# AnyLoc/Revisit-Anything

Hardware: AMD Instinct MI355X
Metric: query_images_per_sec (higher is better)
Workload: dtype f32

## Files before the change

### revisit-anything_amd/csrc/api.hip

```cpp
#include <stdarg.h>
#include <stdlib.h>
#include <string.h>

#include <cmath>
#include <mutex>
#include <utility>

#include <initializer_list>

#include "ctx.h"

int segvlad_ctx::fail(int code, const char* fmt, ...) {
  va_list ap;
  va_start(ap, fmt);
  vsnprintf(err, sizeof(err), fmt, ap);
  va_end(ap);
  return code;
}

bool sv_is_device_ptr(const void* p) {
  hipPointerAttribute_t a;
  memset(&a, 0, sizeof(a));
  hipError_t e = hipPointerGetAttributes(&a, p);
  if (e != hipSuccess) {
// ... 271 lines not shown
  if (!strcmp(key, "f16_gm")) return as_int(&o.f16_gm);
  if (!strcmp(key, "f16_walk")) return as_int(&o.f16_walk);
  if (!strcmp(key, "f16_deep_cfg")) return as_dev(&o.f16_deep_cfg, {-1, 4, 5});
  if (!strcmp(key, "f16_buf")) return as_dev(&o.f16_buf, {-1, 0});
  if (!strcmp(key, "tnk_gram")) return as_int(&o.tnk_gram);
  if (!strcmp(key, "tnk_fork")) return as_int(&o.tnk_fork);
  if (!strcmp(key, "x3_tile")) return as_int(&o.x3_tile);
  if (!strcmp(key, "x3_gm")) return as_int(&o.x3_gm);
  if (!strcmp(key, "search_stats")) return as_int(&o.search_stats);
  if (!strcmp(key, "knn_heuristic")) return as_int(&o.knn_heuristic);
  if (!strcmp(key, "assign_narrow")) return as_int(&o.assign_narrow);
  if (!strcmp(key, "agg_kpb")) return as_int(&o.agg_kpb);
  if (!strcmp(key, "pj_nw")) return as_int(&o.pj_nw);
  if (!strcmp(key, "pj_f16")) return as_int(&o.pj_f16);
  if (!strcmp(key, "cover_rows")) return as_int(&o.cover_rows);
  if (!strcmp(key, "small_plan")) return as_int(&o.small_plan);
  if (!strcmp(key, "small_tail")) return as_int(&o.small_tail);
  if (!strcmp(key, "small_head")) return as_int(&o.small_head);
  if (!strcmp(key, "batch_l0_f16")) return as_int(&o.batch_l0_f16);
  if (!strcmp(key, "level_carry")) return as_int(&o.level_carry);
  if (!strcmp(key, "f16_persist_wgs")) return as_int(&o.f16_persist_wgs);
  if (!strcmp(key, "debug_small_tail")) return as_int(&o.debug_small_tail);
  if (!strcmp(key, "refine_group")) return as_int(&o.refine_group);
  if (!strcmp(key, "query_group")) return as_int(&o.query_group);
  if (!strcmp(key, "group_fetch")) return as_int(&o.group_fetch);
  if (!strcmp(key, "debug_search")) return as_int(&o.debug_search);
  if (!strcmp(key, "debug_fail_search")) return as_int(&o.debug_fail_search);
  if (!strcmp(key, "guard_undersize")) {
    if (!ctx->guard) return ctx->fail(SEGVLAD_ERR_STATE, "set_option(guard_undersize): the context was not created under SEGVLAD_GUARD=1");
    const char* colon = strchr(value, ':');
// ... 353 lines not shown
```

### revisit-anything_amd/csrc/ctx.h

```cpp
#pragma once
#include <hip/hip_runtime.h>
#include <math.h>
#include <stdint.h>
#include <stdio.h>
#include <string.h>

#include <map>
#include <string>
#include <vector>

#include "../../include/segvlad.h"

#define SV_HIP(expr)                                                                              \
  do {                                                                                            \
    hipError_t _e = (expr);                                                                       \
    if (_e != hipSuccess) {                                                                       \
      return ctx->fail(SEGVLAD_ERR_HIP, "%s failed: %s (%s:%d)", #expr, hipGetErrorString(_e),    \
                       __FILE__, __LINE__);                                                       \
    }                                                                                             \
  } while (0)

#define SV_TRY(expr)          \
  do {                        \
    int _r = (expr);          \
// ... 94 lines not shown
  int agg_kpb = 4;
  int debug_fail_search = 0;
  int debug_search = 0;
  int debug_small_tail = 0;
  int batch_l0_f16 = 1;
  int level_carry = 1;
  int small_head = 1;
  int small_tail = 1;
  int small_plan = 1;
  int pj_f16 = 1;
  int pj_nw = 8;
  int refine_group = 1;
  int query_group = 0;
  int pca_path = 0;
  int cover_rows = 1;
  float vlad_soft_temp = 0.f;
  int vlad_soft_pooled = 0;
  int group_fetch = 0;
};

constexpr int SV_F16_KBLOCK = 1024;
inline int sv_f16_kblock(const SvOptions& o, int d) {
  if (o.f16_cfg == 300) return SV_F16_KBLOCK;
  return (o.f16_cfg < 0 && d >= 4096) ? SV_F16_KBLOCK : 0;
}
constexpr int SV_F16_KFLUSH = 64;
int sv_f16_eps_kblock(const SvOptions& o, int d);
inline bool sv_f16_bias_possible(const SvOptions& o, int64_t nq) { return nq > 128 && (o.f16_cfg < 0 || o.f16_cfg == 250 || o.f16_cfg == 300); }
enum class F16Kernel {
  None, BatchDefault, BatchComplement, BatchSmall, BatchUnbiased, BatchUnbiasedSmall, DeepFlush, DeepFlushComplement, DeepBlockedBuf, DeepBlocked,
// ... 269 lines not shown
int sv_launch_refine_grouped(segvlad_ctx* ctx, const float* Q, const float* R, int nq, int d, const float* qn, const float* rn,
                             const uint32_t* ref_cnt, const uint32_t* ref_id, int rcap, int k, float* d2_out, int64_t* idx_out,
                             int* launches, const uint32_t* only_rows = nullptr, int live_groups_hint = 0);
int sv_refine_group_stats(segvlad_ctx* ctx, int nq, int64_t* groups, int64_t* grouped, int64_t* union_sum);
int sv_row_norm_max(segvlad_ctx* ctx, const float* norms, int64_t n, float* out_host, bool finite_only = false);
int sv_row_norm_min(segvlad_ctx* ctx, const float* norms, int64_t n, float* out_host);
int sv_maxabs(segvlad_ctx* ctx, const float* x, int64_t n, float* out_host, bool finite_only = false, bool* nonfinite_host = nullptr);
int sv_maxabs_and_norm_min_begin(segvlad_ctx* ctx, const float* x, int64_t n, const float* norms, int64_t n_norms);
int sv_maxabs_and_norm_min_end(segvlad_ctx* ctx, int64_t n, int64_t n_norms, float* maxabs_host, float* norm_min_host, bool* nonfinite_host,
                               float* norm_max_host);
int sv_launch_split_f16x2(segvlad_ctx* ctx, const float* X, int64_t n_rows, int d, const float* sub, float scale, uint16_t* h1,
                          uint16_t* h2);
int sv_launch_gemm_f16x3(segvlad_ctx* ctx, const uint16_t* A1, const uint16_t* A2, const uint16_t* B1, const uint16_t* B2, int M,
                         int N, int Kd, float out_scale, const float* col_scale, float* C);
int sv_launch_gemm_f16x3_grouped(segvlad_ctx* ctx, const uint16_t* A1, const uint16_t* A2, const uint16_t* B1, const uint16_t* B2,
                                 int M_pad, int N, int Kd, int n_groups, const int32_t* tile_group, float out_scale, float* C);
int sv_launch_group_plan(segvlad_ctx* ctx, const int32_t* cov_cnt, int B, int K, int32_t* rowbase, int32_t* tile_group, int max_tiles);
int sv_launch_project_consts(segvlad_ctx* ctx, const float* comps, const float* mean, int P, int64_t KD, float* wmu );
int sv_launch_project_aggregate(segvlad_ctx* ctx, const float* Z, const float* wmu, const float* block_norms, const float* gscale,
                                const uint64_t* colmask, const int32_t* lab_off, const int32_t* rowbase, const int32_t* phys,
                                const int32_t* seg_off_dev, int B, int N, int K, int P, int SC, int S_max, const float* col_scale,
                                float* Y, float zscale);
int sv_launch_to_f16(segvlad_ctx* ctx, const float* X, int64_t n_elems, float scale, uint16_t* out);
int sv_launch_query_f16_small(segvlad_ctx* ctx, const float* X, int64_t n_elems, float db_scale, uint16_t* out, float* scales_dev,
                              float* qn_out, int nq, int d, uint32_t* zero, int zero_words);
int sv_launch_to_f16_devscale(segvlad_ctx* ctx, const float* X, int64_t n_elems, const float* scales_dev, uint16_t* out);
int sv_launch_f16_filter(segvlad_ctx* ctx, const uint16_t* Qh, const uint16_t* Rh, int M, int n_sample, int d, int b_stride,
                         float inv_scale, const float* qn, const float* rn, const float* thr, int64_t thr_ld, float eps_mult,
                         float c_eps, float rn_max, uint32_t* cand_cnt, float* cand_d2, uint32_t* cand_id, int cap, int skip = 0);
bool sv_f16_filter_skip_ok(const segvlad_ctx* ctx, int M, int64_t n_rows, int d);

int sv_launch_select_cand(segvlad_ctx* ctx, const uint32_t* cand_cnt, const float* cand_d2, const uint32_t* cand_id,
                          int nq, int cap, int k, float* d2_out, int64_t* idx_out, uint32_t* ovf_rows, uint32_t* ovf_count);
int sv_launch_select_topk(segvlad_ctx* ctx, const float* dist, int64_t ld, int nq, int64_t n, int k, float* d2_out,
                          int64_t* idx_out, int64_t out_ld, int64_t id_base);
int sv_launch_merge_topk(segvlad_ctx* ctx, const float* d2_parts, const int64_t* idx_parts, int nq, int cand, int k,
                         float* d2_out, int64_t* idx_out);
// ... 62 lines not shown
```

### revisit-anything_amd/csrc/describe.hip

```cpp
#include <cmath>
#include "ctx.h"


struct SegWalk { int S_max = 0; bool monotone = true; std::vector<int64_t> adj_off; };
static SegWalk walk_seg_offsets(const int32_t* seg_offsets, int B) {
  SegWalk w;
  w.adj_off.assign((size_t)B + 1, 0);
  for (int b = 0; b < B && w.monotone; ++b) {
    const int s = seg_offsets[b + 1] - seg_offsets[b];
    w.monotone = s >= 0;
    if (s > w.S_max) w.S_max = s;
    w.adj_off[b + 1] = w.adj_off[b] + (int64_t)s * s;
  }
  return w;
}

static int incidence_run(segvlad_ctx* ctx, const uint8_t* masks, int S, int Hm, int Wm, int H, int W, int patch, uint64_t* inc_bits,
                         double* centroids, bool want_centroids) {
  if (S < 0 || Hm <= 0 || Wm <= 0 || H <= 0 || W <= 0 || patch <= 0 || H / patch <= 0 || W / patch <= 0)
    return ctx->fail(SEGVLAD_ERR_ARG, "incidence: bad geometry S=%d masks %dx%d image %dx%d patch %d", S, Hm, Wm, H, W, patch);
  if (S == 0) return SEGVLAD_OK;
  if (!masks || !inc_bits || (want_centroids && !centroids)) return ctx->fail(SEGVLAD_ERR_ARG, "incidence: null pointer");
  const int N = (H / patch) * (W / patch), nw = (N + 63) / 64;
  const void* dm;
// ... 121 lines not shown
  p.xscale = sv_fp16_scale(bound);
  p.rows_pad = (((int64_t)B * N + 255) & ~255ll) + 256ll * K;
  if (ctx->pca_w_scale > 0.f) {
    const float zb = std::sqrt((float)D) * (16384.f / ctx->pca_w_scale) * (1.f + ctx->vocab_norm_max);
    if (std::isfinite(zb) && zb > 0.f) p.zscale = sv_fp16_scale(zb);
  }
  return p;
#undef PLAN_REFUSE
}

static int reserve_scratch(segvlad_ctx* ctx, const DescribePlan& p, DescribeIO& io) {
  const size_t B = p.B, N = p.N, D = p.D, K = p.K, P = p.P, S = p.S_tot;
  if (p.form == DescribeForm::Project) {
    SV_HIP(ctx->s_xh1.reserve((size_t)(p.rows_pad + 256) * D * 2));
    SV_HIP(ctx->s_xh2.reserve((size_t)(p.rows_pad + 256) * D * 2));
    SV_HIP(ctx->s_pz.reserve((size_t)p.rows_pad * P * sizeof(float)));
    SV_HIP(ctx->s_rowbase.reserve(B * K * sizeof(int32_t)));
    SV_HIP(ctx->s_tilegrp.reserve((size_t)(p.rows_pad >> 8) * sizeof(int32_t)));
    SV_HIP(ctx->s_phys.reserve(B * N * sizeof(int32_t)));
    SV_HIP(ctx->s_covcnt.reserve(B * K * sizeof(int32_t)));
    SV_HIP(ctx->s_bn.reserve(S * K * sizeof(float)));
  } else if (p.form == DescribeForm::Planes) {
    SV_HIP(ctx->s_xh1.reserve((size_t)sv_x3_rows(p.S_tot) * ctx->KD * 2));
    SV_HIP(ctx->s_xh2.reserve((size_t)sv_x3_rows(p.S_tot) * ctx->KD * 2));
  } else if (p.form == DescribeForm::PlainProjection && !io.out && S > 0) {
    SV_HIP(ctx->s_desc.reserve(S * ctx->KD * sizeof(float)));
    io.out = ctx->s_desc.as<float>();
  }
  SV_HIP(ctx->s_xt.reserve(B * N * D * sizeof(float)));
  SV_HIP(ctx->s_rnorm.reserve(B * N * sizeof(float)));
  if (!p.want_labels) SV_HIP(ctx->s_labels.reserve(B * N));
// ... 100 lines not shown
}

static int pass_project(segvlad_ctx* ctx, const DescribePlan& p, const DescribeIO& io) {
  float* bn = io.d_bn ? (float*)io.d_bn : ctx->s_bn.as<float>();
  uint16_t *h1 = ctx->s_xh1.as<uint16_t>(), *h2 = ctx->s_xh2.as<uint16_t>();
  {
    StageScope sc(ctx, "aggregate");
    SV_TRY(sv_launch_group_plan(ctx, ctx->s_covcnt.as<int32_t>(), p.B, p.K, ctx->s_rowbase.as<int32_t>(), ctx->s_tilegrp.as<int32_t>(),
                                (int)(p.rows_pad >> 8)));
    SV_TRY(sv_launch_token_norms(ctx, ctx->s_xt.as<float>(), ctx->s_colmask.as<uint64_t>(), ctx->vocab.as<float>(), p.K, p.D,
                                 ctx->s_segoff.as<int32_t>(), p.B, p.N, p.SC, bn, p.xscale, h1, h2, ctx->s_rowbase.as<int32_t>(),
                                 ctx->opt.debug_search == 7 ? -p.rows_pad : p.rows_pad, ctx->s_phys.as<int32_t>()));
    sc.count(2);
  }
  StageScope sc(ctx, "pca");
  SV_TRY(sv_launch_gemm_f16x3_grouped(ctx, h1, h2, ctx->pca_w1.as<uint16_t>(), ctx->pca_w2.as<uint16_t>(), (int)p.rows_pad, p.P, p.D, p.K,
                                      ctx->s_tilegrp.as<int32_t>(), 1.f / (p.xscale * ctx->pca_w_scale), ctx->s_pz.as<float>()));
  SV_TRY(sv_launch_project_aggregate(ctx, ctx->s_pz.as<float>(), ctx->pca_cproj.as<float>(), bn, ctx->s_gscale.as<float>(),
                                     ctx->s_colmask.as<uint64_t>(), ctx->s_laboff.as<int32_t>(), ctx->s_rowbase.as<int32_t>(),
                                     ctx->s_phys.as<int32_t>(), ctx->s_segoff.as<int32_t>(), p.B, p.N, p.K, p.P, p.SC, p.S_max,
                                     ctx->pca_scale.as<float>(), (float*)io.d_y, p.zscale));
  sc.count(2);
  return pass_normalize(ctx, p, io, sc);
}

static int join_mask_branch(segvlad_ctx* ctx) {
  if (!ctx->desc.side_pending) return SEGVLAD_OK;
  ctx->desc.side_pending = false;
  return sv_join_side(ctx);
}
static int run_describe(segvlad_ctx* ctx, const DescribePlan& p, DescribeIO& io) {
  SV_TRY(reserve_scratch(ctx, p, io));
  if (p.form == DescribeForm::Project && !ctx->pca_cproj_valid) {
    SV_HIP(ctx->pca_cproj.reserve((size_t)ctx->P * sizeof(float)));
    SV_TRY(sv_launch_project_consts(ctx, ctx->pca_comps.as<float>(), ctx->pca_mean.as<float>(), ctx->P, ctx->KD, ctx->pca_cproj.as<float>()));
    ctx->pca_cproj_valid = true;
// ... 284 lines not shown
```

### revisit-anything_amd/csrc/gemm_f16x3_kernels.hip

```cpp
#include <stdlib.h>

#include "ctx.h"

typedef float f32x4 __attribute__((ext_vector_type(4)));
typedef _Float16 f16x8 __attribute__((ext_vector_type(8)));
typedef const __attribute__((address_space(1))) void* gptr_t;
typedef __attribute__((address_space(3))) void* lptr_t;
#define MFMA_F16(a, b, c) __builtin_amdgcn_mfma_f32_16x16x32_f16((a), (b), (c), 0, 0, 0)

__global__ __launch_bounds__(256) void split_f16x2_kernel(const float* __restrict__ X, int64_t n_rows, int d,
                                                          const float* __restrict__ sub, float scale,
                                                          _Float16* __restrict__ h1, _Float16* __restrict__ h2) {
  typedef _Float16 h4 __attribute__((ext_vector_type(4)));
  const int64_t n4 = n_rows * (int64_t)(d >> 2);
  const int d4 = d >> 2;
  for (int64_t j = (int64_t)blockIdx.x * 256 + threadIdx.x; j < n4; j += (int64_t)gridDim.x * 256) {
    float4 v = reinterpret_cast<const float4*>(X)[j];
    if (sub) {
      const float4 s = reinterpret_cast<const float4*>(sub)[j % d4];
      v.x -= s.x;
      v.y -= s.y;
      v.z -= s.z;
      v.w -= s.w;
    }
// ... 25 lines not shown
__device__ __forceinline__ void wait_vm_lgkm0_() {
  if (N_ == 0) asm volatile("s_waitcnt vmcnt(0) lgkmcnt(0)" ::: "memory");
  else if (N_ == 2) asm volatile("s_waitcnt vmcnt(2) lgkmcnt(0)" ::: "memory");
  else if (N_ == 4) asm volatile("s_waitcnt vmcnt(4) lgkmcnt(0)" ::: "memory");
  else asm volatile("s_waitcnt vmcnt(8) lgkmcnt(0)" ::: "memory");
}

template <int BM, int BN, int WM, int WN>
__global__ __launch_bounds__(64 * WM * WN) void gemm_f16x3_kernel(const uint16_t* __restrict__ A1,
                                                                  const uint16_t* __restrict__ A2,
                                                                  const uint16_t* __restrict__ B1,
                                                                  const uint16_t* __restrict__ B2, int M, int N, int Kd,
                                                                  int tiles_m, int gm, int n_splits, int k_per_split, float out_scale,
                                                                  const float* __restrict__ col_scale,
                                                                  float* __restrict__ C, int64_t ldc,
                                                                  const int32_t* __restrict__ tile_group, int nkb_b) {
  constexpr int NW = WM * WN;
  constexpr int TM = BM / (16 * WM), TN = BN / (16 * WN);
  static_assert(TM == 4 && (TN == 8 || TN == 4), "wave tiles of 64 rows, 128 or 64 columns");
  constexpr int HBK = 32, RB = 64, RP = 16;
  constexpr int PA = BM * RB, PB = BN * RB;
  constexpr int JA = BM / RP / NW, JB = BN / RP / NW;
  static_assert(JA * RP * NW == BM && JB * RP * NW == BN, "tile/wave geometry");
  extern __shared__ __attribute__((aligned(16))) unsigned char lds[];
  int tm, tn, split;
  if (gm > 0) {
    const int b = blockIdx.x, xcd = b & 7, s = b >> 3, within = s & 31, u = (s >> 5) * 8 + xcd;
    const int gn = 32 / gm, sm_cnt = (tiles_m + gm - 1) / gm, tiles_n = (N + BN - 1) / BN;
    split = u % n_splits;
    const int r = u / n_splits;
    tm = (r % sm_cnt) * gm + within % gm;
// ... 102 lines not shown
#pragma unroll
        for (int nt = 0; nt < 4; ++nt) acc[mt][4 * h + nt] = MFMA_F16(a1[mt], b1[nt], acc[mt][4 * h + nt]);
    }
    wait_vm_lgkm0_<0>();
    __builtin_amdgcn_s_barrier();
    cur ^= 1;
  }

  if (n_splits > 1) C += (int64_t)split * M * ldc;
#pragma unroll
  for (int nt = 0; nt < TN; ++nt) {
    const int64_t col = n0 + wn * (16 * TN) + nt * 16 + i;
    if (col >= N) continue;
    const float cs = (n_splits > 1) ? 1.f : out_scale * (col_scale ? col_scale[col] : 1.f);
#pragma unroll
    for (int mt = 0; mt < TM; ++mt)
#pragma unroll
      for (int r = 0; r < 4; ++r) {
        const int64_t row = m0 + wm * (16 * TM) + mt * 16 + 4 * kq + r;
        if (row < M) C[row * ldc + col] = acc[mt][nt][r] * cs;
      }
  }
}

__global__ __launch_bounds__(256) void splitk_reduce_scale_kernel(const float* __restrict__ part, int splits, int64_t mn,
                                                                  int N, float out_scale,
                                                                  const float* __restrict__ col_scale,
                                                                  float* __restrict__ out) {
  const int64_t j = (int64_t)blockIdx.x * 256 + threadIdx.x;
  if (j >= mn) return;
  float s = part[j];
  for (int t = 1; t < splits; ++t) s += part[(int64_t)t * mn + j];
  const int col = (int)(j % N);
  out[j] = s * out_scale * (col_scale ? col_scale[col] : 1.f);
}

// ... 25 lines not shown
  const size_t lds = 2 * (size_t)(2 * BM * 64 + 2 * BN * 64);
  auto kern = gemm_f16x3_kernel<BM, BN, WM, WN>;
  if (lds > 64 * 1024)
    SV_HIP(sv_max_dyn_lds(reinterpret_cast<const void*>(kern), (size_t)lds));
  int gm = ctx->opt.x3_gm > 0 ? ctx->opt.x3_gm : 0;
  dim3 grid((unsigned)tiles, (unsigned)splits);
  if (gm > 0) {
    gm = gm >= 32 ? 32 : gm >= 16 ? 16 : gm >= 8 ? 8 : gm >= 4 ? 4 : gm >= 2 ? 2 : 1;
    while (gm < 32 && 32 / gm > tiles_n) gm <<= 1;
    while (gm > 1 && gm / 2 >= tiles_m) gm >>= 1;
    const int gn = 32 / gm;
    const int64_t units = (int64_t)((tiles_m + gm - 1) / gm) * ((tiles_n + gn - 1) / gn) * splits;
    grid = dim3((unsigned)((units + 7) / 8 * 8 * 32), 1);
  }
  hipLaunchKernelGGL(kern, grid, dim3(64 * WM * WN), lds, ctx->stream, A1, A2, B1, B2, M, N, Kd, tiles_m, gm, splits, k_per_split,
                     out_scale, col_scale, dst, (int64_t)N, (const int32_t*)nullptr, 0);
  SV_HIP(hipGetLastError());
  if (splits > 1) {
    const int64_t mn = (int64_t)M * N;
    hipLaunchKernelGGL(splitk_reduce_scale_kernel, dim3((unsigned)((mn + 255) / 256)), dim3(256), 0, ctx->stream, dst, splits, mn,
                       N, out_scale, col_scale, C);
    SV_HIP(hipGetLastError());
  }
  return SEGVLAD_OK;
}

int sv_launch_gemm_f16x3(segvlad_ctx* ctx, const uint16_t* A1, const uint16_t* A2, const uint16_t* B1, const uint16_t* B2, int M,
                         int N, int Kd, float out_scale, const float* col_scale, float* C) {
  if (M <= 0 || N <= 0) return SEGVLAD_OK;
  const bool big = ctx->opt.x3_tile ? (ctx->opt.x3_tile == 256) : (M >= 1024);
  if (big) return launch_x3<256, 256, 4, 2>(ctx, A1, A2, B1, B2, M, N, Kd, out_scale, col_scale, C);
  return launch_x3<128, 128, 2, 2>(ctx, A1, A2, B1, B2, M, N, Kd, out_scale, col_scale, C);
}

int sv_launch_gemm_f16x3_grouped(segvlad_ctx* ctx, const uint16_t* A1, const uint16_t* A2, const uint16_t* B1, const uint16_t* B2,
                                 int M_pad, int N, int Kd, int n_groups, const int32_t* tile_group, float out_scale, float* C) {
  if (M_pad <= 0 || N <= 0) return SEGVLAD_OK;
  constexpr int BM = 256, BN = 256;
  const int tiles_m = M_pad / BM, tiles_n = (N + BN - 1) / BN;
  const size_t lds = 2 * (size_t)(2 * BM * 64 + 2 * BN * 64);
  auto kern = gemm_f16x3_kernel<BM, BN, 4, 2>;
  SV_HIP(sv_max_dyn_lds(reinterpret_cast<const void*>(kern), (size_t)lds));
  const int rows_per_chunk = 32 / tiles_n > 0 ? 32 / tiles_n : 1;
  const int chunks = (tiles_m + rows_per_chunk - 1) / rows_per_chunk;
  const int64_t grid = (int64_t)((chunks + 7) / 8) * 8 * rows_per_chunk * tiles_n;
  hipLaunchKernelGGL(kern, dim3((unsigned)grid, 1), dim3(512), lds, ctx->stream, A1, A2, B1, B2, M_pad, N, Kd, tiles_m, 0,
                     1, Kd, out_scale, (const float*)nullptr, C, (int64_t)N, tile_group, n_groups * (Kd >> 5));
  SV_HIP(hipGetLastError());
  return SEGVLAD_OK;
}
```

### revisit-anything_amd/csrc/project_kernels.hip

```cpp
#include "ctx.h"
#include "group_tile_dev.h"

#define MFMA32(a, b, c) __builtin_amdgcn_mfma_f32_32x32x2f32((a), (b), (c), 0, 0, 0)

__global__ __launch_bounds__(1024) void group_plan_kernel(const int32_t* __restrict__ cov_cnt, int B, int K,
                                                          int32_t* __restrict__ rowbase, int32_t* __restrict__ tile_group,
                                                          int max_tiles) {
  __shared__ int32_t part[1024], base[257];
  const int nsl = 1024 / K;
  const int k = threadIdx.x % K, c = threadIdx.x / K;
  const int per = (B + nsl - 1) / nsl, b0 = c * per, b1 = min(B, b0 + per);
  const bool act = c < nsl;
  for (int t = threadIdx.x; t < max_tiles; t += blockDim.x) tile_group[t] = -1;
  int sum = 0;
  if (act)
    for (int b = b0; b < b1; ++b) sum += cov_cnt[(size_t)b * K + k];
  part[threadIdx.x] = act ? sum : 0;
  __syncthreads();
  if ((int)threadIdx.x < K) {
    int run = 0;
    for (int q = 0; q < nsl; ++q) {
      const int v = part[q * K + threadIdx.x];
      part[q * K + threadIdx.x] = run;
      run += v;
// ... 38 lines not shown
  for (int o = 128; o > 0; o >>= 1) {
    if ((int)threadIdx.x < o) red[threadIdx.x] += red[threadIdx.x + o];
    __syncthreads();
  }
  if (threadIdx.x == 0) wmu[p] = (float)red[0];
}

int sv_launch_project_consts(segvlad_ctx* ctx, const float* comps, const float* mean, int P, int64_t KD, float* wmu) {
  hipLaunchKernelGGL(project_consts_kernel, dim3(P), dim3(256), 0, ctx->stream, comps, mean, P, KD, wmu);
  SV_HIP(hipGetLastError());
  return SEGVLAD_OK;
}

constexpr int PJ_T = 32;

template <int NW, bool F16 = false>
__global__ __launch_bounds__(64 * NW) void project_aggregate_kernel(const float* __restrict__ Z, const float* __restrict__ wmu,
                                                                const float* __restrict__ bn, const float* __restrict__ gscale,
                                                                const uint64_t* __restrict__ colmask,
                                                                const int32_t* __restrict__ lab_off,
                                                                const int32_t* __restrict__ rowbase,
                                                                const int32_t* __restrict__ phys,
                                                                const int32_t* __restrict__ seg_off, int N, int K, int P, int SC,
                                                                int maxt, const float* __restrict__ col_scale,
                                                                float* __restrict__ Y, float zscale) {
  extern __shared__ __attribute__((aligned(16))) unsigned char smem[];
  typedef _Float16 f16x8 __attribute__((ext_vector_type(8)));
  static_assert(!F16 || NW == 8, "16-bit tile sums: the 8-wave workgroup");
  const int KS = K + 1 + (K & 1);
  float* ag = reinterpret_cast<float*>(smem);
  constexpr int NC = 32 * NW, NT_ = 64 * NW, C4W = NC / 4;
  float* zt = ag + 64 * KS;
  uint64_t* mk = reinterpret_cast<uint64_t*>(zt + 2 * PJ_T * NC);
  int32_t* tl_k = reinterpret_cast<int32_t*>(mk + 2 * PJ_T);
  int32_t* tl_j = tl_k + maxt;
  int32_t* tl_z = tl_j + maxt;
  int32_t* tl_n = tl_z + maxt;
  int32_t* phl = tl_n + maxt + K + 1;
  uint4* af = reinterpret_cast<uint4*>((reinterpret_cast<uintptr_t>(phl + N) + 15) & ~(uintptr_t)15);
  __shared__ int s_tiles;
  const int b = blockIdx.y, p0 = blockIdx.x * NC;
  const int tid = threadIdx.x, w = tid >> 6, l = tid & 63, i = l & 31, kk = l >> 5;
  const int s0 = seg_off[b], S = seg_off[b + 1] - s0;
  const int SCb = (S + 63) >> 6;
  const int32_t* lo = lab_off + (size_t)b * (K + 1);
  const int pcol = p0 + 32 * w + i;
  int32_t* tl_pre = tl_n + maxt;
  int my_o0 = 0, my_n = 0, my_g0 = 0;
  if (tid < K) {
    my_o0 = lo[tid];
    my_n = lo[tid + 1] - my_o0;
    my_g0 = rowbase[(size_t)b * K + tid];
    tl_pre[tid + 1] = (my_n + PJ_T - 1) / PJ_T;
  }
// ... 8 lines not shown
    }
    s_tiles = run < maxt ? run : maxt;
  }
  __syncthreads();
  if (tid < K) {
    int t = tl_pre[tid];
    for (int j0 = 0; j0 < my_n && t < maxt; j0 += PJ_T, ++t) {
      tl_k[t] = tid;
      tl_j[t] = my_o0 + j0;
      tl_z[t] = my_g0;
      tl_n[t] = min(PJ_T, my_n - j0);
    }
  }
  __syncthreads();
  const int tiles = s_tiles;

  for (int sc = 0; sc < SCb; ++sc) {
    const int Sc = min(64, S - 64 * sc);
    __syncthreads();
    for (int idx = tid; idx < 64 * K; idx += NT_) {
      const int s = idx / K, k = idx - s * K;
      float a = 0.f;
      if (s < Sc) {
        const float nrm = bn[(size_t)(s0 + 64 * sc + s) * K + k];
        a = nrm > 1e-12f ? gscale[s0 + 64 * sc + s] / nrm : 0.f;
      }
      if (F16) ag[k * 64 + s] = a;
      else ag[s * KS + k] = a;
    }
    f32x16 acc[2];
// ... 52 lines not shown
      const float a0k = ag[i * KS + k_], a1k = ag[(32 + i) * KS + k_];                                          \
      const float* ztc = zt + (size_t)cur_ * PJ_T * NC + 32 * w + i;                                            \
      const uint64_t* mkc = mk + cur_ * PJ_T;                                                                   \
      for (int pr = 0; 2 * pr < nt_; ++pr) {                                                                    \
        const int j = 2 * pr + kk;                                                                              \
        const uint64_t m = mkc[j];                                                                              \
        const float bv = ztc[j * NC];                                                                           \
        const float a0 = ((m >> i) & 1ull) ? a0k : 0.f;                                                         \
        acc[0] = MFMA32(a0, bv, acc[0]);                                                                        \
        if (two) {                                                                                              \
          const float a1 = ((m >> (32 + i)) & 1ull) ? a1k : 0.f;                                                \
          acc[1] = MFMA32(a1, bv, acc[1]);                                                                      \
        }                                                                                                       \
      }                                                                                                         \
    } while (0)
#define SV_PJ_MUL16(t_)                                                                                         \
    do {                                                                                                        \
      const int cur_ = (t_) & 1, k_ = tl_k[t_], nt_ = tl_n[t_];                                                 \
      const float* ztc = zt + (size_t)cur_ * PJ_T * NC + 32 * w + i + (size_t)(8 * kk) * NC;                    \
      const uint4* afc = af + cur_ * 256 + l;                                                                   \
      f32x16 ta0, ta1;                                                                                          \
      _Pragma("unroll") for (int ks = 0; ks < 2; ++ks) {                                                        \
        if (ks == 1 && nt_ <= 16) break;                                                                        \
        f16x8 hh, ll;                                                                                           \
        _Pragma("unroll") for (int e = 0; e < 8; ++e) {                                                         \
          const float v = ztc[(size_t)(16 * ks + e) * NC] * zscale;                                             \
          hh[e] = (_Float16)v;                                                                                  \
          ll[e] = (_Float16)(v - (float)hh[e]);                                                                 \
        }                                                                                                       \
        const uint4 a0u = afc[(2 * ks) * 64];                                                                   \
        const f16x8 a0 = __builtin_bit_cast(f16x8, a0u);                                                        \
        if (ks == 0) {                                                                                          \
          f32x16 zero_;                                                                                         \
          _Pragma("unroll") for (int r = 0; r < 16; ++r) zero_[r] = 0.f;                                        \
          ta0 = __builtin_amdgcn_mfma_f32_32x32x16_f16(a0, ll, zero_, 0, 0, 0);                                 \
        } else {                                                                                                \
          ta0 = __builtin_amdgcn_mfma_f32_32x32x16_f16(a0, ll, ta0, 0, 0, 0);                                   \
        }                                                                                                       \
        ta0 = __builtin_amdgcn_mfma_f32_32x32x16_f16(a0, hh, ta0, 0, 0, 0);                                     \
        if (two) {                                                                                              \
          const uint4 a1u = afc[(2 * ks + 1) * 64];                                                             \
          const f16x8 a1 = __builtin_bit_cast(f16x8, a1u);                                                      \
          if (ks == 0) {                                                                                        \
            f32x16 zero_;                                                                                       \
// ... 12 lines not shown
        acc[0][4 * q + 0] = fmaf(w0.x, ta0[4 * q + 0], acc[0][4 * q + 0]);                                      \
        acc[0][4 * q + 1] = fmaf(w0.y, ta0[4 * q + 1], acc[0][4 * q + 1]);                                      \
        acc[0][4 * q + 2] = fmaf(w0.z, ta0[4 * q + 2], acc[0][4 * q + 2]);                                      \
        acc[0][4 * q + 3] = fmaf(w0.w, ta0[4 * q + 3], acc[0][4 * q + 3]);                                      \
        if (two) {                                                                                              \
          const float4 w1 = *reinterpret_cast<const float4*>(agk + 32 + 8 * q);                                 \
          acc[1][4 * q + 0] = fmaf(w1.x, ta1[4 * q + 0], acc[1][4 * q + 0]);                                    \
          acc[1][4 * q + 1] = fmaf(w1.y, ta1[4 * q + 1], acc[1][4 * q + 1]);                                    \
          acc[1][4 * q + 2] = fmaf(w1.z, ta1[4 * q + 2], acc[1][4 * q + 2]);                                    \
          acc[1][4 * q + 3] = fmaf(w1.w, ta1[4 * q + 3], acc[1][4 * q + 3]);                                    \
        }                                                                                                       \
      }                                                                                                         \
    } while (0)
#define SV_PJ_MULX(t_)                                                                                          \
    do {                                                                                                        \
      if constexpr (F16) SV_PJ_MUL16(t_);                                                                       \
      else SV_PJ_MUL(t_);                                                                                       \
    } while (0)
    if (tiles > 0) {
      SV_PJ_FETCH(va, ma, 0);
      SV_PJ_FETCH_F(fa, 0);
      SV_PJ_STASH(va, ma, 0);
      SV_PJ_STASH_F(fa, 0);
    }
    if (tiles > 1) {
      SV_PJ_FETCH(va, ma, 1);
      SV_PJ_FETCH_F(fa, 1);
    }
    __syncthreads();
    for (int t = 0; t < tiles; t += 2) {
      if (t + 2 < tiles) {
        SV_PJ_FETCH(vb, mb, t + 2);
        SV_PJ_FETCH_F(fb, t + 2);
// ... 4 lines not shown
        SV_PJ_STASH_F(fa, 1);
      }
      __syncthreads();
      if (t + 1 >= tiles) break;
      if (t + 3 < tiles) {
        SV_PJ_FETCH(va, ma, t + 3);
        SV_PJ_FETCH_F(fa, t + 3);
      }
      SV_PJ_MULX(t + 1);
      if (t + 2 < tiles) {
        SV_PJ_STASH(vb, mb, 0);
        SV_PJ_STASH_F(fb, 0);
      }
      __syncthreads();
    }
#undef SV_PJ_MULX
#undef SV_PJ_MUL16
#undef SV_PJ_STASH_F
#undef SV_PJ_FETCH_F
#undef SV_PJ_MUL
#undef SV_PJ_STASH
#undef SV_PJ_FETCH
    if (pcol < P) {
      const float cs = col_scale ? col_scale[pcol] : 1.f, mu = wmu[pcol];
#pragma unroll
      for (int mt = 0; mt < 2; ++mt) {
        if (mt == 1 && !two) break;
#pragma unroll
        for (int r = 0; r < 16; ++r) {
          const int s = 32 * mt + sv_frag_row(r, kk);
          if (s < Sc) Y[(size_t)(s0 + 64 * sc + s) * P + pcol] = ((F16 ? acc[mt][r] * (1.f / zscale) : acc[mt][r]) - mu) * cs;
        }
      }
    }
  }
}

int sv_launch_project_aggregate(segvlad_ctx* ctx, const float* Z, const float* wmu, const float* block_norms, const float* gscale,
                                const uint64_t* colmask, const int32_t* lab_off, const int32_t* rowbase, const int32_t* phys,
                                const int32_t* seg_off_dev, int B, int N, int K, int P, int SC, int S_max, const float* col_scale,
                                float* Y, float zscale) {
  if (B <= 0 || S_max <= 0) return SEGVLAD_OK;
  if (P % 4) return ctx->fail(SEGVLAD_ERR_ARG, "project_aggregate: P=%d must be a multiple of 4", P);
  const int maxt = K + (N + PJ_T - 1) / PJ_T;
  const int nw = ctx->opt.pj_nw == 4 ? 4 : 8;
  if (K > 64 * nw) return ctx->fail(SEGVLAD_ERR_LIMIT, "project_aggregate: K=%d clusters need %d threads", K, K);
  const bool f16 = zscale > 0.f && nw == 8 && ctx->opt.pj_f16 != 0;
  const size_t lds = (size_t)64 * (K + 1 + (K & 1)) * 4 + (size_t)2 * PJ_T * 32 * nw * 4 + (size_t)2 * PJ_T * 8 + (size_t)4 * maxt * 4 +
                     (size_t)(K + 1) * 4 + (size_t)N * 4 + (f16 ? 16 + 2 * 256 * 16 : 0);
  if (lds > 160 * 1024)
    return ctx->fail(SEGVLAD_ERR_LIMIT, "project_aggregate: K=%d, N=%d need %zu B of LDS", K, N, lds);
  const void* fn = f16 ? reinterpret_cast<const void*>(project_aggregate_kernel<8, true>)
                       : nw == 8 ? reinterpret_cast<const void*>(project_aggregate_kernel<8>) : reinterpret_cast<const void*>(project_aggregate_kernel<4>);
  if (lds > 64 * 1024) SV_HIP(sv_max_dyn_lds(fn, (size_t)lds));
  const dim3 grid((P + 32 * nw - 1) / (32 * nw), B), block(64 * nw);
  if (f16)
    hipLaunchKernelGGL((project_aggregate_kernel<8, true>), grid, block, lds, ctx->stream, Z, wmu, block_norms, gscale, colmask, lab_off,
                       rowbase, phys, seg_off_dev, N, K, P, SC, maxt, col_scale, Y, zscale);
  else if (nw == 8)
    hipLaunchKernelGGL(project_aggregate_kernel<8>, grid, block, lds, ctx->stream, Z, wmu, block_norms, gscale, colmask, lab_off, rowbase,
                       phys, seg_off_dev, N, K, P, SC, maxt, col_scale, Y, 0.f);
  else
    hipLaunchKernelGGL(project_aggregate_kernel<4>, grid, block, lds, ctx->stream, Z, wmu, block_norms, gscale, colmask, lab_off, rowbase,
                       phys, seg_off_dev, N, K, P, SC, maxt, col_scale, Y, 0.f);
  SV_HIP(hipGetLastError());
  return SEGVLAD_OK;
}
```

Measured before the change: 8768.

## Emit Z as packed fp16 hi/lo pairs from PCA GEMM and load them directly in aggregation

The grouped PCA GEMM epilogue now scales each output by zscale and writes it as packed fp16 high/low pairs instead of fp32. The project-aggregate kernel gains a ZP variant that loads these pairs straight from global memory into registers, using precomputed per-tile row offsets held in LDS and a three-stage register pipeline. This removes the LDS staging of Z tiles and the per-element fp16 split inside the inner loop. In exchange it needs an extra zeroed padding row, a memset, 32-bit byte-offset indexing (guarded by a size check), and a more complex prefetch schedule.

```diff
diff --git a/revisit-anything_amd/csrc/api.hip b/revisit-anything_amd/csrc/api.hip
--- a/revisit-anything_amd/csrc/api.hip
+++ b/revisit-anything_amd/csrc/api.hip
@@ -309,6 +309,7 @@
   if (!strcmp(key, "pj_nw")) return as_int(&o.pj_nw);
   if (!strcmp(key, "pj_f16")) return as_int(&o.pj_f16);
   if (!strcmp(key, "cover_rows")) return as_int(&o.cover_rows);
+  if (!strcmp(key, "pj_planes")) return as_int(&o.pj_planes);
   if (!strcmp(key, "small_plan")) return as_int(&o.small_plan);
   if (!strcmp(key, "small_tail")) return as_int(&o.small_tail);
   if (!strcmp(key, "small_head")) return as_int(&o.small_head);
diff --git a/revisit-anything_amd/csrc/ctx.h b/revisit-anything_amd/csrc/ctx.h
--- a/revisit-anything_amd/csrc/ctx.h
+++ b/revisit-anything_amd/csrc/ctx.h
@@ -132,6 +132,7 @@
   int query_group = 0;
   int pca_path = 0;
   int cover_rows = 1;
+  int pj_planes = 1;
   float vlad_soft_temp = 0.f;
   int vlad_soft_pooled = 0;
   int group_fetch = 0;
@@ -431,13 +432,15 @@
 int sv_launch_gemm_f16x3(segvlad_ctx* ctx, const uint16_t* A1, const uint16_t* A2, const uint16_t* B1, const uint16_t* B2, int M,
                          int N, int Kd, float out_scale, const float* col_scale, float* C);
 int sv_launch_gemm_f16x3_grouped(segvlad_ctx* ctx, const uint16_t* A1, const uint16_t* A2, const uint16_t* B1, const uint16_t* B2,
-                                 int M_pad, int N, int Kd, int n_groups, const int32_t* tile_group, float out_scale, float* C);
+                                 int M_pad, int N, int Kd, int n_groups, const int32_t* tile_group, float out_scale, float* C,
+                                 float pair_scale);
 int sv_launch_group_plan(segvlad_ctx* ctx, const int32_t* cov_cnt, int B, int K, int32_t* rowbase, int32_t* tile_group, int max_tiles);
 int sv_launch_project_consts(segvlad_ctx* ctx, const float* comps, const float* mean, int P, int64_t KD, float* wmu );
+bool sv_project_z_pairs(const segvlad_ctx* ctx, float zscale, int64_t rows, int P);
 int sv_launch_project_aggregate(segvlad_ctx* ctx, const float* Z, const float* wmu, const float* block_norms, const float* gscale,
                                 const uint64_t* colmask, const int32_t* lab_off, const int32_t* rowbase, const int32_t* phys,
                                 const int32_t* seg_off_dev, int B, int N, int K, int P, int SC, int S_max, const float* col_scale,
-                                float* Y, float zscale);
+                                float* Y, float zscale, int z_pairs, int64_t zero_row);
 int sv_launch_to_f16(segvlad_ctx* ctx, const float* X, int64_t n_elems, float scale, uint16_t* out);
 int sv_launch_query_f16_small(segvlad_ctx* ctx, const float* X, int64_t n_elems, float db_scale, uint16_t* out, float* scales_dev,
                               float* qn_out, int nq, int d, uint32_t* zero, int zero_words);
diff --git a/revisit-anything_amd/csrc/describe.hip b/revisit-anything_amd/csrc/describe.hip
--- a/revisit-anything_amd/csrc/describe.hip
+++ b/revisit-anything_amd/csrc/describe.hip
@@ -159,7 +159,7 @@
   if (p.form == DescribeForm::Project) {
     SV_HIP(ctx->s_xh1.reserve((size_t)(p.rows_pad + 256) * D * 2));
     SV_HIP(ctx->s_xh2.reserve((size_t)(p.rows_pad + 256) * D * 2));
-    SV_HIP(ctx->s_pz.reserve((size_t)p.rows_pad * P * sizeof(float)));
+    SV_HIP(ctx->s_pz.reserve((size_t)(p.rows_pad + 1) * P * sizeof(float)));
     SV_HIP(ctx->s_rowbase.reserve(B * K * sizeof(int32_t)));
     SV_HIP(ctx->s_tilegrp.reserve((size_t)(p.rows_pad >> 8) * sizeof(int32_t)));
     SV_HIP(ctx->s_phys.reserve(B * N * sizeof(int32_t)));
@@ -290,12 +290,16 @@
     sc.count(2);
   }
   StageScope sc(ctx, "pca");
+  const bool z_pairs = sv_project_z_pairs(ctx, p.zscale, p.rows_pad + 1, p.P);
+  if (z_pairs)
+    SV_HIP(hipMemsetAsync(ctx->s_pz.as<float>() + (size_t)p.rows_pad * p.P, 0, (size_t)p.P * sizeof(float), ctx->stream));
   SV_TRY(sv_launch_gemm_f16x3_grouped(ctx, h1, h2, ctx->pca_w1.as<uint16_t>(), ctx->pca_w2.as<uint16_t>(), (int)p.rows_pad, p.P, p.D, p.K,
-                                      ctx->s_tilegrp.as<int32_t>(), 1.f / (p.xscale * ctx->pca_w_scale), ctx->s_pz.as<float>()));
+                                      ctx->s_tilegrp.as<int32_t>(), 1.f / (p.xscale * ctx->pca_w_scale), ctx->s_pz.as<float>(),
+                                      z_pairs ? p.zscale : 0.f));
   SV_TRY(sv_launch_project_aggregate(ctx, ctx->s_pz.as<float>(), ctx->pca_cproj.as<float>(), bn, ctx->s_gscale.as<float>(),
                                      ctx->s_colmask.as<uint64_t>(), ctx->s_laboff.as<int32_t>(), ctx->s_rowbase.as<int32_t>(),
                                      ctx->s_phys.as<int32_t>(), ctx->s_segoff.as<int32_t>(), p.B, p.N, p.K, p.P, p.SC, p.S_max,
-                                     ctx->pca_scale.as<float>(), (float*)io.d_y, p.zscale));
+                                     ctx->pca_scale.as<float>(), (float*)io.d_y, p.zscale, z_pairs ? 1 : 0, p.rows_pad));
   sc.count(2);
   return pass_normalize(ctx, p, io, sc);
 }
diff --git a/revisit-anything_amd/csrc/gemm_f16x3_kernels.hip b/revisit-anything_amd/csrc/gemm_f16x3_kernels.hip
--- a/revisit-anything_amd/csrc/gemm_f16x3_kernels.hip
+++ b/revisit-anything_amd/csrc/gemm_f16x3_kernels.hip
@@ -63,7 +63,8 @@
                                                                   int tiles_m, int gm, int n_splits, int k_per_split, float out_scale,
                                                                   const float* __restrict__ col_scale,
                                                                   float* __restrict__ C, int64_t ldc,
-                                                                  const int32_t* __restrict__ tile_group, int nkb_b) {
+                                                                  const int32_t* __restrict__ tile_group, int nkb_b,
+                                                                  float pair_scale) {
   constexpr int NW = WM * WN;
   constexpr int TM = BM / (16 * WM), TN = BN / (16 * WN);
   static_assert(TM == 4 && (TN == 8 || TN == 4), "wave tiles of 64 rows, 128 or 64 columns");
@@ -196,12 +197,28 @@
     if (col >= N) continue;
     const float cs = (n_splits > 1) ? 1.f : out_scale * (col_scale ? col_scale[col] : 1.f);
 #pragma unroll
-    for (int mt = 0; mt < TM; ++mt)
-#pragma unroll
-      for (int r = 0; r < 4; ++r) {
-        const int64_t row = m0 + wm * (16 * TM) + mt * 16 + 4 * kq + r;
-        if (row < M) C[row * ldc + col] = acc[mt][nt][r] * cs;
+    for (int mt = 0; mt < TM; ++mt) {
+      const int64_t row0 = m0 + wm * (16 * TM) + mt * 16 + 4 * kq;
+      if (pair_scale > 0.f) {
+        typedef float f32x2 __attribute__((ext_vector_type(2)));
+        typedef _Float16 f16x2 __attribute__((ext_vector_type(2)));
+#pragma unroll
+        for (int r = 0; r < 4; r += 2) {
+          const f32x2 z = {acc[mt][nt][r] * cs, acc[mt][nt][r + 1] * cs};
+          const f32x2 v = z * pair_scale;
+          const f16x2 h = __builtin_convertvector(v, f16x2);
+          const f16x2 lo = __builtin_convertvector(v - __builtin_convertvector(h, f32x2), f16x2);
+          const uint32_t hu = __builtin_bit_cast(uint32_t, h), lu = __builtin_bit_cast(uint32_t, lo);
+          uint32_t* dst = reinterpret_cast<uint32_t*>(C) + (row0 + r) * ldc + col;
+          if (row0 + r < M) dst[0] = (hu & 0xffffu) | (lu << 16);
+          if (row0 + r + 1 < M) dst[ldc] = (hu >> 16) | (lu & 0xffff0000u);
+        }
+      } else {
+#pragma unroll
+        for (int r = 0; r < 4; ++r)
+          if (row0 + r < M) C[(row0 + r) * ldc + col] = acc[mt][nt][r] * cs;
       }
+    }
   }
 }
 
@@ -257,7 +274,7 @@
     grid = dim3((unsigned)((units + 7) / 8 * 8 * 32), 1);
   }
   hipLaunchKernelGGL(kern, grid, dim3(64 * WM * WN), lds, ctx->stream, A1, A2, B1, B2, M, N, Kd, tiles_m, gm, splits, k_per_split,
-                     out_scale, col_scale, dst, (int64_t)N, (const int32_t*)nullptr, 0);
+                     out_scale, col_scale, dst, (int64_t)N, (const int32_t*)nullptr, 0, 0.f);
   SV_HIP(hipGetLastError());
   if (splits > 1) {
     const int64_t mn = (int64_t)M * N;
@@ -277,7 +294,8 @@
 }
 
 int sv_launch_gemm_f16x3_grouped(segvlad_ctx* ctx, const uint16_t* A1, const uint16_t* A2, const uint16_t* B1, const uint16_t* B2,
-                                 int M_pad, int N, int Kd, int n_groups, const int32_t* tile_group, float out_scale, float* C) {
+                                 int M_pad, int N, int Kd, int n_groups, const int32_t* tile_group, float out_scale, float* C,
+                                 float pair_scale) {
   if (M_pad <= 0 || N <= 0) return SEGVLAD_OK;
   constexpr int BM = 256, BN = 256;
   const int tiles_m = M_pad / BM, tiles_n = (N + BN - 1) / BN;
@@ -288,7 +306,7 @@
   const int chunks = (tiles_m + rows_per_chunk - 1) / rows_per_chunk;
   const int64_t grid = (int64_t)((chunks + 7) / 8) * 8 * rows_per_chunk * tiles_n;
   hipLaunchKernelGGL(kern, dim3((unsigned)grid, 1), dim3(512), lds, ctx->stream, A1, A2, B1, B2, M_pad, N, Kd, tiles_m, 0,
-                     1, Kd, out_scale, (const float*)nullptr, C, (int64_t)N, tile_group, n_groups * (Kd >> 5));
+                     1, Kd, out_scale, (const float*)nullptr, C, (int64_t)N, tile_group, n_groups * (Kd >> 5), pair_scale);
   SV_HIP(hipGetLastError());
   return SEGVLAD_OK;
 }
diff --git a/revisit-anything_amd/csrc/project_kernels.hip b/revisit-anything_amd/csrc/project_kernels.hip
--- a/revisit-anything_amd/csrc/project_kernels.hip
+++ b/revisit-anything_amd/csrc/project_kernels.hip
@@ -76,7 +76,7 @@
 
 constexpr int PJ_T = 32;
 
-template <int NW, bool F16 = false>
+template <int NW, bool F16 = false, bool ZP = false>
 __global__ __launch_bounds__(64 * NW) void project_aggregate_kernel(const float* __restrict__ Z, const float* __restrict__ wmu,
                                                                 const float* __restrict__ bn, const float* __restrict__ gscale,
                                                                 const uint64_t* __restrict__ colmask,
@@ -85,21 +85,23 @@
                                                                 const int32_t* __restrict__ phys,
                                                                 const int32_t* __restrict__ seg_off, int N, int K, int P, int SC,
                                                                 int maxt, const float* __restrict__ col_scale,
-                                                                float* __restrict__ Y, float zscale) {
+                                                                float* __restrict__ Y, float zscale, int64_t zrow) {
   extern __shared__ __attribute__((aligned(16))) unsigned char smem[];
   typedef _Float16 f16x8 __attribute__((ext_vector_type(8)));
   static_assert(!F16 || NW == 8, "16-bit tile sums: the 8-wave workgroup");
+  static_assert(!ZP || F16, "fp16 pairs of Z: the 16-bit tile sums");
   const int KS = K + 1 + (K & 1);
   float* ag = reinterpret_cast<float*>(smem);
   constexpr int NC = 32 * NW, NT_ = 64 * NW, C4W = NC / 4;
   float* zt = ag + 64 * KS;
-  uint64_t* mk = reinterpret_cast<uint64_t*>(zt + 2 * PJ_T * NC);
+  uint64_t* mk = reinterpret_cast<uint64_t*>(zt + (ZP ? 0 : 2 * PJ_T * NC));
   int32_t* tl_k = reinterpret_cast<int32_t*>(mk + 2 * PJ_T);
   int32_t* tl_j = tl_k + maxt;
   int32_t* tl_z = tl_j + maxt;
   int32_t* tl_n = tl_z + maxt;
   int32_t* phl = tl_n + maxt + K + 1;
-  uint4* af = reinterpret_cast<uint4*>((reinterpret_cast<uintptr_t>(phl + N) + 15) & ~(uintptr_t)15);
+  uint4* af = reinterpret_cast<uint4*>(smem + ((size_t)(reinterpret_cast<unsigned char*>(phl + N) - smem + 15) & ~(size_t)15));
+  uint32_t* tro = reinterpret_cast<uint32_t*>(af + 3 * 256);
   __shared__ int s_tiles;
   const int b = blockIdx.y, p0 = blockIdx.x * NC;
   const int tid = threadIdx.x, w = tid >> 6, l = tid & 63, i = l & 31, kk = l >> 5;
@@ -138,6 +140,18 @@
   }
   __syncthreads();
   const int tiles = s_tiles;
+  if constexpr (ZP) {
+    const uint32_t zoff = (uint32_t)zrow * (uint32_t)P * 4u;
+    for (int idx = tid; idx < (tiles + 1) * PJ_T; idx += NT_) {
+      const int t = idx / PJ_T, r = idx % PJ_T;
+      uint32_t o = zoff;
+      if (t < tiles && r < tl_n[t]) {
+        const int pr = phl[tl_j[t] + r];
+        if (pr >= 0) o = (uint32_t)(tl_z[t] + pr) * (uint32_t)P * 4u;
+      }
+      tro[idx] = o;
+    }
+  }
 
   for (int sc = 0; sc < SCb; ++sc) {
     const int Sc = min(64, S - 64 * sc);
@@ -220,20 +234,35 @@
         }                                                                                                       \
       }                                                                                                         \
     } while (0)
-#define SV_PJ_MUL16(t_)                                                                                         \
-    do {                                                                                                        \
-      const int cur_ = (t_) & 1, k_ = tl_k[t_], nt_ = tl_n[t_];                                                 \
-      const float* ztc = zt + (size_t)cur_ * PJ_T * NC + 32 * w + i + (size_t)(8 * kk) * NC;                    \
-      const uint4* afc = af + cur_ * 256 + l;                                                                   \
+#define SV_PJ_HL_SPLIT(cur_, V_, ks, hh, ll)                                                                    \
+    do {                                                                                                        \
+      const float* ztc = zt + (size_t)(cur_) * PJ_T * NC + 32 * w + i + (size_t)(8 * kk) * NC;                  \
+      _Pragma("unroll") for (int e = 0; e < 8; ++e) {                                                           \
+        const float v = ztc[(size_t)(16 * (ks) + e) * NC] * zscale;                                             \
+        hh[e] = (_Float16)v;                                                                                    \
+        ll[e] = (_Float16)(v - (float)hh[e]);                                                                   \
+      }                                                                                                         \
+    } while (0)
+#define SV_PJ_HL_PAIRS(cur_, V_, ks, hh, ll)                                                                    \
+    do {                                                                                                        \
+      uint32_t hd_[4], ld_[4];                                                                                  \
+      _Pragma("unroll") for (int m = 0; m < 4; ++m) {                                                           \
+        const uint32_t e0_ = V_[8 * (ks) + 2 * m], e1_ = V_[8 * (ks) + 2 * m + 1];                              \
+        hd_[m] = (e0_ & 0xffffu) | (e1_ << 16);                                                                 \
+        ld_[m] = (e0_ >> 16) | (e1_ & 0xffff0000u);                                                             \
+      }                                                                                                         \
+      hh = __builtin_bit_cast(f16x8, make_uint4(hd_[0], hd_[1], hd_[2], hd_[3]));                               \
+      ll = __builtin_bit_cast(f16x8, make_uint4(ld_[0], ld_[1], ld_[2], ld_[3]));                               \
+    } while (0)
+#define SV_PJ_MUL16(t_, cur_, HL_, V_)                                                                          \
+    do {                                                                                                        \
+      const int k_ = tl_k[t_], nt_ = tl_n[t_];                                                                  \
+      const uint4* afc = af + (cur_) * 256 + l;                                                                 \
       f32x16 ta0, ta1;                                                                                          \
       _Pragma("unroll") for (int ks = 0; ks < 2; ++ks) {                                                        \
         if (ks == 1 && nt_ <= 16) break;                                                                        \
         f16x8 hh, ll;                                                                                           \
-        _Pragma("unroll") for (int e = 0; e < 8; ++e) {                                                         \
-          const float v = ztc[(size_t)(16 * ks + e) * NC] * zscale;                                             \
-          hh[e] = (_Float16)v;                                                                                  \
-          ll[e] = (_Float16)(v - (float)hh[e]);                                                                 \
-        }                                                                                                       \
+        HL_(cur_, V_, ks, hh, ll);                                                                              \
         const uint4 a0u = afc[(2 * ks) * 64];                                                                   \
         const f16x8 a0 = __builtin_bit_cast(f16x8, a0u);                                                        \
         if (ks == 0) {                                                                                          \
@@ -276,9 +305,64 @@
     } while (0)
 #define SV_PJ_MULX(t_)                                                                                          \
     do {                                                                                                        \
-      if constexpr (F16) SV_PJ_MUL16(t_);                                                                       \
+      if constexpr (F16) SV_PJ_MUL16(t_, (t_) & 1, SV_PJ_HL_SPLIT, va);                                         \
       else SV_PJ_MUL(t_);                                                                                       \
     } while (0)
+#define SV_PZ_FETCH(V, t_)                                                                                      \
+    do {                                                                                                        \
+      const uint4* tr_ = reinterpret_cast<const uint4*>(tro + ((t_) < tiles ? (t_) : tiles) * PJ_T + 8 * kk);   \
+      const uint4 o0_ = tr_[0], o1_ = tr_[1], o2_ = tr_[4], o3_ = tr_[5];                                       \
+      const uint32_t o_[16] = {o0_.x, o0_.y, o0_.z, o0_.w, o1_.x, o1_.y, o1_.z, o1_.w,                          \
+                               o2_.x, o2_.y, o2_.z, o2_.w, o3_.x, o3_.y, o3_.z, o3_.w};                         \
+      _Pragma("unroll") for (int q = 0; q < 16; ++q)                                                            \
+        V[q] = *reinterpret_cast<const uint32_t*>(reinterpret_cast<const unsigned char*>(Z) + (o_[q] + col4));  \
+    } while (0)
+#define SV_PZ_FETCH_M(Mv, t_)                                                                                   \
+    do {                                                                                                        \
+      const int tt_ = (t_) < tiles ? (t_) : tiles - 1;                                                          \
+      const int j0_ = 16 * (tid >> 8) + 8 * ((tid >> 5) & 1) + 4 * ((tid >> 6) & 1);                            \
+      const int nt_ = ((t_) < tiles ? tl_n[tt_] : 0) - j0_;                                                     \
+      const uint32_t* zero_ = reinterpret_cast<const uint32_t*>(Z) + (size_t)zrow * P;                          \
+      const uint32_t* mrow_ = reinterpret_cast<const uint32_t*>(colmask + ((size_t)b * N + tl_j[tt_] + j0_) * SC + sc) + ((tid >> 7) & 1); \
+      _Pragma("unroll") for (int q = 0; q < 4; ++q) Mv[q] = *(q < nt_ ? mrow_ + (size_t)q * SC * 2 : zero_); \
+    } while (0)
+#define SV_PZ_STASH_M(Mv, slot_)                                                                                \
+    do {                                                                                                        \
+      const int sh_ = tid & 31;                                                                                 \
+      uint2 d_;                                                                                                 \
+      d_.x = (((Mv[0] >> sh_) & 1u) ? 0x3C00u : 0u) | (((Mv[1] >> sh_) & 1u) ? 0x3C000000u : 0u);               \
+      d_.y = (((Mv[2] >> sh_) & 1u) ? 0x3C00u : 0u) | (((Mv[3] >> sh_) & 1u) ? 0x3C000000u : 0u);               \
+      reinterpret_cast<uint2*>(af + (slot_) * 256 + (tid >> 7) * 64 + (tid & 63))[(tid >> 6) & 1] = d_;         \
+    } while (0)
+#define SV_PZ_STEP(Vc, sc_, Mn, sn_, V2, M2, t_)                                                                \
+    do {                                                                                                        \
+      SV_PZ_FETCH_M(M2, (t_) + 2);                                                                              \
+      SV_PZ_FETCH(V2, (t_) + 2);                                                                                \
+      SV_PJ_MUL16(t_, sc_, SV_PJ_HL_PAIRS, Vc);                                                                 \
+      SV_PZ_STASH_M(Mn, sn_);                                                                                   \
+      __syncthreads();                                                                                          \
+    } while (0)
+    if constexpr (ZP) {
+      if (tiles > 0) {
+        const uint32_t col4 = 4u * (uint32_t)(pcol < P ? pcol : P - 1);
+        uint32_t za[16], zb[16], zc[16], ma_[4], mb_[4], mc_[4];
+        SV_PZ_FETCH_M(ma_, 0);
+        SV_PZ_FETCH(za, 0);
+        SV_PZ_FETCH_M(mb_, 1);
+        SV_PZ_FETCH(zb, 1);
+        SV_PZ_STASH_M(ma_, 0);
+        __syncthreads();
+        for (int t = 0; t < tiles; t += 3) {
+          SV_PZ_STEP(za, 0, mb_, 1, zc, mc_, t);
+          if (t + 1 >= tiles) break;
+          SV_PZ_STEP(zb, 1, mc_, 2, za, ma_, t + 1);
+          if (t + 2 >= tiles) break;
+          SV_PZ_STEP(zc, 2, ma_, 0, zb, mb_, t + 2);
+        }
+      } else {
+        __syncthreads();
+      }
+    } else {
     if (tiles > 0) {
       SV_PJ_FETCH(va, ma, 0);
       SV_PJ_FETCH_F(fa, 0);
@@ -313,8 +397,15 @@
       }
       __syncthreads();
     }
+    }
+#undef SV_PZ_STEP
+#undef SV_PZ_STASH_M
+#undef SV_PZ_FETCH_M
+#undef SV_PZ_FETCH
 #undef SV_PJ_MULX
 #undef SV_PJ_MUL16
+#undef SV_PJ_HL_PAIRS
+#undef SV_PJ_HL_SPLIT
 #undef SV_PJ_STASH_F
 #undef SV_PJ_FETCH_F
 #undef SV_PJ_MUL
@@ -335,33 +426,43 @@
   }
 }
 
+bool sv_project_z_pairs(const segvlad_ctx* ctx, float zscale, int64_t rows, int P) {
+  return zscale > 0.f && ctx->opt.pj_nw != 4 && ctx->opt.pj_f16 != 0 && ctx->opt.pj_planes != 0 && rows * P * 4 < (1ll << 32);
+}
+
 int sv_launch_project_aggregate(segvlad_ctx* ctx, const float* Z, const float* wmu, const float* block_norms, const float* gscale,
                                 const uint64_t* colmask, const int32_t* lab_off, const int32_t* rowbase, const int32_t* phys,
                                 const int32_t* seg_off_dev, int B, int N, int K, int P, int SC, int S_max, const float* col_scale,
-                                float* Y, float zscale) {
+                                float* Y, float zscale, int z_pairs, int64_t zero_row) {
   if (B <= 0 || S_max <= 0) return SEGVLAD_OK;
   if (P % 4) return ctx->fail(SEGVLAD_ERR_ARG, "project_aggregate: P=%d must be a multiple of 4", P);
   const int maxt = K + (N + PJ_T - 1) / PJ_T;
   const int nw = ctx->opt.pj_nw == 4 ? 4 : 8;
   if (K > 64 * nw) return ctx->fail(SEGVLAD_ERR_LIMIT, "project_aggregate: K=%d clusters need %d threads", K, K);
   const bool f16 = zscale > 0.f && nw == 8 && ctx->opt.pj_f16 != 0;
-  const size_t lds = (size_t)64 * (K + 1 + (K & 1)) * 4 + (size_t)2 * PJ_T * 32 * nw * 4 + (size_t)2 * PJ_T * 8 + (size_t)4 * maxt * 4 +
-                     (size_t)(K + 1) * 4 + (size_t)N * 4 + (f16 ? 16 + 2 * 256 * 16 : 0);
+  if (z_pairs && !sv_project_z_pairs(ctx, zscale, zero_row + 1, P)) return ctx->fail(SEGVLAD_ERR_STATE, "project_aggregate: fp16 pairs of Z without the 16-bit tile sums");
+  const size_t lds = (size_t)64 * (K + 1 + (K & 1)) * 4 + (z_pairs ? 0 : (size_t)2 * PJ_T * 32 * nw * 4) + (size_t)2 * PJ_T * 8 +
+                     (size_t)4 * maxt * 4 + (size_t)(K + 1) * 4 + (size_t)N * 4 + (f16 ? 16 + (z_pairs ? 3 : 2) * 256 * 16 : 0) +
+                     (z_pairs ? (size_t)(maxt + 1) * PJ_T * 4 : 0);
   if (lds > 160 * 1024)
     return ctx->fail(SEGVLAD_ERR_LIMIT, "project_aggregate: K=%d, N=%d need %zu B of LDS", K, N, lds);
-  const void* fn = f16 ? reinterpret_cast<const void*>(project_aggregate_kernel<8, true>)
+  const void* fn = z_pairs ? reinterpret_cast<const void*>(project_aggregate_kernel<8, true, true>)
+                   : f16 ? reinterpret_cast<const void*>(project_aggregate_kernel<8, true>)
                        : nw == 8 ? reinterpret_cast<const void*>(project_aggregate_kernel<8>) : reinterpret_cast<const void*>(project_aggregate_kernel<4>);
   if (lds > 64 * 1024) SV_HIP(sv_max_dyn_lds(fn, (size_t)lds));
   const dim3 grid((P + 32 * nw - 1) / (32 * nw), B), block(64 * nw);
-  if (f16)
+  if (z_pairs)
+    hipLaunchKernelGGL((project_aggregate_kernel<8, true, true>), grid, block, lds, ctx->stream, Z, wmu, block_norms, gscale, colmask, lab_off,
+                       rowbase, phys, seg_off_dev, N, K, P, SC, maxt, col_scale, Y, zscale, zero_row);
+  else if (f16)
     hipLaunchKernelGGL((project_aggregate_kernel<8, true>), grid, block, lds, ctx->stream, Z, wmu, block_norms, gscale, colmask, lab_off,
-                       rowbase, phys, seg_off_dev, N, K, P, SC, maxt, col_scale, Y, zscale);
+                       rowbase, phys, seg_off_dev, N, K, P, SC, maxt, col_scale, Y, zscale, (int64_t)0);
   else if (nw == 8)
     hipLaunchKernelGGL(project_aggregate_kernel<8>, grid, block, lds, ctx->stream, Z, wmu, block_norms, gscale, colmask, lab_off, rowbase,
-                       phys, seg_off_dev, N, K, P, SC, maxt, col_scale, Y, 0.f);
+                       phys, seg_off_dev, N, K, P, SC, maxt, col_scale, Y, 0.f, (int64_t)0);
   else
     hipLaunchKernelGGL(project_aggregate_kernel<4>, grid, block, lds, ctx->stream, Z, wmu, block_norms, gscale, colmask, lab_off, rowbase,
-                       phys, seg_off_dev, N, K, P, SC, maxt, col_scale, Y, 0.f);
+                       phys, seg_off_dev, N, K, P, SC, maxt, col_scale, Y, 0.f, (int64_t)0);
   SV_HIP(hipGetLastError());
   return SEGVLAD_OK;
 }
```

After: 8857 (median of 6 runs). +1.0%, better.
